# tenpy/cyten

Measured on AMD Instinct MI355X. Metric: block-sparse tdot+SVD GFLOP/s (fp64), higher is better.
Workload: dtype f64

## Files before the change

cyten_amd/csrc/jacobi_engine.hip:

```cpp
#include "jacobi_engine.h"
#include "jacobi_plan.h"

#include <algorithm>
#include <cmath>
#include <cstdlib>

namespace cyb {
namespace {

typedef double d4 __attribute__((ext_vector_type(4)));
typedef double d2 __attribute__((ext_vector_type(2)));
#define GLOBAL_AS __attribute__((address_space(1)))
typedef const GLOBAL_AS d2* gc2;
typedef const GLOBAL_AS d2* gcp2;
typedef GLOBAL_AS double* gp;

constexpr int GS = JP + 2;
constexpr int QS = JP + 16;
constexpr int GK = 64;
constexpr int XS = GK + 2;
constexpr int NT = 256;
constexpr int NPAIR = JP / 2;
static_assert(JP == 32, "the wave tiling below assumes 32 x 32 pair problems");

// ... 513 lines not shown
                double* Xr = which ? Ur : Hr;
                double* Xi = which ? Ui : Hi;
                const double c = rot[k * 4], sn = rot[k * 4 + 1], fr = rot[k * 4 + 2], fi = -rot[k * 4 + 3];
                const double pr_ = Xr[row * CS + p], pi_ = Xi[row * CS + p], qr_ = Xr[row * CS + q], qi_ = Xi[row * CS + q];
                const double tr = fr * qr_ - fi * qi_, ti = fr * qi_ + fi * qr_;
                Xr[row * CS + p] = c * pr_ - sn * tr;
                Xi[row * CS + p] = c * pi_ - sn * ti;
                Xr[row * CS + q] = sn * pr_ + c * tr;
                Xi[row * CS + q] = sn * pi_ + c * ti;
            }
            __builtin_amdgcn_fence(__ATOMIC_RELEASE, "wavefront");
            __builtin_amdgcn_wave_barrier();
        }
    for (int e = lane; e < CJ * CJ; e += 64) {
        const int a = e / CJ, b = e % CJ;
        const double x = Ur[a * CS + b], y = Ui[a * CS + b];
        Vout[(2 * a) * VS + 2 * b] = x;
        Vout[(2 * a) * VS + 2 * b + 1] = -y;
        Vout[(2 * a + 1) * VS + 2 * b] = y;
        Vout[(2 * a + 1) * VS + 2 * b + 1] = x;
    }
    if (lane < CJ) {
        const double lam = Hr[lane * CS + lane];
        Gdiag[(2 * lane) * GS + 2 * lane] = lam;
        Gdiag[(2 * lane + 1) * GS + 2 * lane + 1] = lam;
    }
}

struct SScratch {
    double* gpart;
    unsigned int* ticket;
    unsigned int* ready;
    unsigned int* err;
    const int2* wgmap;
    const int2* wgent;
    unsigned long long* stamps;
    int stamp_round;
    int n_sweeps, n_mats;
    unsigned int* arrive;
    int* nsw;
    unsigned int* readyJ;
    int defer_j;
    unsigned long long* gran;
    int gran_np;
    int cross_every, cross_min_nb;
};
constexpr int SW_MAX_ENT = 64;

constexpr int SW_UN = 8;
constexpr int SW_PRE = 6;
constexpr int SW_GRAN_U64 = 2 * JP * JP;
constexpr unsigned int SW_GRAN_BYTES = 8u * SW_GRAN_U64;
static_assert(SW_GRAN_BYTES == kPlanGranBytes, "granule regions of jacobi_plan.h");
constexpr int SWEEP_XREG = (4 * JP * GS > JP * GS + 2 * JP * VS) ? 4 * JP * GS : JP * GS + 2 * JP * VS;
constexpr int SWEEP_LDS_DOUBLES = JP * GS + SWEEP_XREG + 2 * JP * QS + 8;
constexpr size_t SWEEP_LDS_BYTES = 88 * 1024;
static_assert((size_t)SWEEP_LDS_DOUBLES * 8 + 1024 <= SWEEP_LDS_BYTES, "LDS request of the sweep kernel");
constexpr int SWEEP_WG_PER_CU = 1;

typedef unsigned int u32x2 __attribute__((ext_vector_type(2)));
union Q8 {
    u32x2 u;
    double d;
};

template <int SLEEP = 1>
__device__ __forceinline__ bool spin_until(const unsigned int* word, unsigned int target, unsigned int* err)
{
    const unsigned long long t0 = wall_clock64();
    unsigned int it = 0;
    while (__hip_atomic_load(word, __ATOMIC_RELAXED, __HIP_MEMORY_SCOPE_AGENT) < target) {
        __builtin_amdgcn_s_sleep(SLEEP);
        if ((++it & 63u) == 0u) {
            if (__hip_atomic_load(err, __ATOMIC_RELAXED, __HIP_MEMORY_SCOPE_AGENT) != 0u) return false;
            if (wall_clock64() - t0 > 100000000ull) {
                __hip_atomic_store(err, 1u, __ATOMIC_RELAXED, __HIP_MEMORY_SCOPE_AGENT);
                return false;
            }
        }
    }
    return true;
}

template <int SLEEP = 1>
__device__ __forceinline__ bool spin_until2(const unsigned int* word0, const unsigned int* word1, unsigned int target, unsigned int* err)
{
    const unsigned long long t0 = wall_clock64();
    unsigned int it = 0;
    for (;;) {
        const unsigned int v0 = __hip_atomic_load(word0, __ATOMIC_RELAXED, __HIP_MEMORY_SCOPE_AGENT);
        const unsigned int v1 = __hip_atomic_load(word1, __ATOMIC_RELAXED, __HIP_MEMORY_SCOPE_AGENT);
        if ((v0 >= target) & (v1 >= target)) return true;
        __builtin_amdgcn_s_sleep(SLEEP);
        if ((++it & 63u) == 0u) {
            if (__hip_atomic_load(err, __ATOMIC_RELAXED, __HIP_MEMORY_SCOPE_AGENT) != 0u) return false;
            if (wall_clock64() - t0 > 100000000ull) {
                __hip_atomic_store(err, 1u, __ATOMIC_RELAXED, __HIP_MEMORY_SCOPE_AGENT);
                return false;
            }
        }
    }
}
template <bool RORD>
__device__ __forceinline__ bool spin_pair(const unsigned int* word0, const unsigned int* word1, unsigned int target, unsigned int* err)
{
    if constexpr (RORD) return spin_until2(word0, word1, target, err);
    else return spin_until(word0, target, err) && spin_until(word1, target, err);
}

__device__ __forceinline__ void sweep_update_j(const __amdgpu_buffer_rsrc_t rsJ, const double* Qm, int P, int Q, int nvp, int j_begin,
                                               int nJ, int wave, int lane)
{
    const int un = lane & 15, ukq = lane >> 4;
    const double* ap0 = Qm + (lane >> 4) * QS + (lane & 15);
    const double* ap1 = ap0 + 16;
    double a0[JP / 4], a1[JP / 4];
#pragma unroll
    for (int kk = 0; kk < JP / 4; ++kk) {
        a0[kk] = ap0[kk * 4 * QS];
        a1[kk] = ap1[kk * 4 * QS];
    }
    auto off_of = [&](int c, int k) { return (unsigned int)(((int64_t)xrow(k, P, Q) * nvp + (j_begin + c) * 64 + wave * 16 + un) * 8); };
    auto load = [&](double (&x)[JP / 4], int c) {
#pragma unroll
        for (int kk = 0; kk < JP / 4; ++kk) {
            Q8 q;
            q.u = __builtin_amdgcn_raw_buffer_load_b64(rsJ, off_of(c, 4 * kk + ukq), 0, 16);
            x[kk] = q.d;
        }
    };
    double xb[JP / 4], xn[JP / 4];
    if (nJ > 0) load(xb, 0);
    for (int c = 0; c < nJ; ++c) {
        if (c + 1 < nJ) load(xn, c + 1);
        d4 acc[2] = {d4{0.0, 0.0, 0.0, 0.0}, d4{0.0, 0.0, 0.0, 0.0}};
#pragma unroll
        for (int kk = 0; kk < JP / 4; ++kk) {
            acc[0] = __builtin_amdgcn_mfma_f64_16x16x4f64(a0[kk], xb[kk], acc[0], 0, 0, 0);
            acc[1] = __builtin_amdgcn_mfma_f64_16x16x4f64(a1[kk], xb[kk], acc[1], 0, 0, 0);
        }
#pragma unroll
        for (int i = 0; i < 2; ++i)
#pragma unroll
            for (int q = 0; q < 4; ++q) {
                Q8 v;
                v.d = acc[i][q];
                __builtin_amdgcn_raw_buffer_store_b64(v.u, rsJ, off_of(c, i * 16 + (lane >> 4) + 4 * q), 0, 16);
            }
#pragma unroll
        for (int kk = 0; kk < JP / 4; ++kk) xb[kk] = xn[kk];
    }
}

template <bool CPLX, bool RORD, bool GRAN>
__global__ void __launch_bounds__(NT, 1)
jacobi_sweep_kernel(const RPair* __restrict__ pairs, int max_inner, unsigned long long* __restrict__ offmax_bits, SScratch sc)
{
    extern __shared__ __attribute__((aligned(16))) double rsm[];
    double* Gs = rsm;
    double* G2 = Gs + JP * GS;
    double* Va = G2 + JP * GS;
    double* Vb = Va + JP * VS;
    double* Xc = G2;
    double* Qs0 = G2 + SWEEP_XREG;
    double* Qs1 = Qs0 + JP * QS;
    double* red = Qs1 + JP * QS;
    int* ibase = reinterpret_cast<int*>(red + 8);
    int* perm = ibase;
    int* zrow = ibase + JP;
    int* zout = ibase + 2 * JP;
    int* flags = ibase + 3 * JP;
    int* edone = flags + 4;

    const int tid = threadIdx.x;
    const int lane = tid & 63, wave = tid >> 6;
    const int2 went = sc.wgent ? sc.wgent[blockIdx.x] : make_int2((int)blockIdx.x, (int)blockIdx.x + 1);
    int max_rounds = 0;
    for (int e = went.x; e < went.y; ++e) max_rounds = max(max_rounds, pairs[sc.wgmap[e].x].nb - 1);
    const int n_sw = sc.n_sweeps;
    const bool one_entry = went.y - went.x == 1;
    int pendP = -1, pendQ = -1, pend_ground = 0;
    if (n_sw > 1) {
        if (tid < SW_MAX_ENT) edone[tid] = 0;
        __syncthreads();
    }
    for (int sw = 0; sw < n_sw; ++sw) {
    for (int round = 0; round < max_rounds; ++round)
    for (int ent = went.x; ent < went.y; ++ent) {
    const int2 wm = sc.wgmap[ent];
    const int pi = wm.x, part = wm.y;
    const RPair mt = pairs[pi];
    if (round >= mt.nb - 1) continue;
    if (n_sw > 1 && edone[ent - went.x]) continue;
    const int ground = sw * (mt.nb - 1) + round;
    const int G = mt.pad[0];
    unsigned int* ready = sc.ready + mt.pad[1];
    unsigned int* readyJ = sc.readyJ + mt.pad[1];
    unsigned int* ticket = sc.ticket + pi;
    double* Qs = (ground & 1) ? Qs1 : Qs0;
    const unsigned int pbytes = JP * JP * 8;
    const __amdgpu_buffer_rsrc_t rsW = __builtin_amdgcn_make_buffer_rsrc(mt.W, 0, (int)((size_t)mt.nvp * mt.lenp * 8), 0x00020000);
    const __amdgpu_buffer_rsrc_t rsJ =
        __builtin_amdgcn_make_buffer_rsrc(mt.J ? mt.J : mt.W, 0, mt.J ? (int)((size_t)mt.nvp * mt.nvp * 8) : 0, 0x00020000);
    const int cw = mt.lenp / 64, cj = mt.J ? mt.nvp / 64 : 0;
    const int w_begin = (int)((int64_t)part * cw / G), w_end = (int)((int64_t)(part + 1) * cw / G);
    const int j_begin = (int)((int64_t)part * cj / G), j_end = (int)((int64_t)(part + 1) * cj / G);
    const int nW = w_end - w_begin, nJ = j_end - j_begin;
    const bool defer = sc.defer_j && one_entry && G > 1 && nJ > 0 && round < mt.nb - 2;
    const int ct = defer ? nW : nW + nJ;
    const int pre_limit = (sc.defer_j && G > 1) ? min(ct, nW) : ct;
    const int un = lane & 15, ukq = lane >> 4;
#define SWEEP_STAMP(k)                                                                                            \
    do {                                                                                                          \
        if (sc.stamps && tid == 0 && round == sc.stamp_round) sc.stamps[(size_t)blockIdx.x * 8 + (k)] = wall_clock64(); \
    } while (0)

    {
        int P, Q;
        circle_pair(mt.nb, round, mt.slot, P, Q);
        if (P > Q) {
            const int t = P;
            P = Q;
            Q = t;
        }
        SWEEP_STAMP(0);
        __syncthreads();
        if (ground > 0) {
            if (tid == 0) {
                flags[1] = spin_pair<RORD>(ready + (size_t)P * G + part, ready + (size_t)Q * G + part, (unsigned int)ground, sc.err) ? 1 : 0;
            }
            __syncthreads();
            if (!flags[1]) return;
        }
        SWEEP_STAMP(1);
        if constexpr (GRAN) {
            if (tid == 0) flags[3] = 0;
        }
        auto chunk_off = [&](int c, int k, bool& in_w) -> unsigned int {
            in_w = c < nW;
            const int ld = in_w ? mt.lenp : mt.nvp;
            const int cc = in_w ? w_begin + c : j_begin + (c - nW);
            return (unsigned int)(((int64_t)xrow(k, P, Q) * ld + cc * 64 + wave * 16 + un) * 8);
        };
        auto chunk_load = [&](int c, int k) -> double {
            bool in_w;
            const unsigned int off = chunk_off(c, k, in_w);
            Q8 q;
            q.u = in_w ? __builtin_amdgcn_raw_buffer_load_b64(rsW, off, 0, 16) : __builtin_amdgcn_raw_buffer_load_b64(rsJ, off, 0, 16);
            return q.d;
        };
        double xpre[SW_PRE][JP / 4];
        auto issue_xpre = [&]() {
#pragma unroll
            for (int c = 0; c < SW_PRE; ++c) {
                if (c < pre_limit) {
#pragma unroll
                    for (int kk = 0; kk < JP / 4; ++kk) xpre[c][kk] = chunk_load(c, 4 * kk + ukq);
                }
            }
        };
        {
            const int ld = mt.lenp;
            d4 acc00 = d4{0.0, 0.0, 0.0, 0.0}, acc01 = acc00, acc11 = acc00;
            const int r = lane & 15, g2 = 2 * (lane >> 4);
            const unsigned int o0 = (unsigned int)(((int64_t)xrow(r, P, Q) * ld + g2) * 8);
            const unsigned int o1 = (unsigned int)(((int64_t)xrow(r + 16, P, Q) * ld + g2) * 8);
            const int c_begin = 8 * w_begin, c_end = 8 * w_end;
            constexpr int UN = SW_UN;
            d2 x0[UN], x1[UN], n0[UN], n1[UN];
            auto load = [&](d2 (&a0)[UN], d2 (&a1)[UN], int c0) {
#pragma unroll
                for (int u = 0; u < UN; ++u) {
                    const int c = min(c0 + 4 * u, c_end - 1);
                    Q16 qa, qb;
                    qa.u = __builtin_amdgcn_raw_buffer_load_b128(rsW, o0 + (unsigned int)c * 64u, 0, 16);
                    qb.u = __builtin_amdgcn_raw_buffer_load_b128(rsW, o1 + (unsigned int)c * 64u, 0, 16);
                    a0[u] = qa.d;
                    a1[u] = qb.d;
                }
            };
            auto gram = [&](const d2 (&a0)[UN], const d2 (&a1)[UN], int c0) {
#pragma unroll
                for (int u = 0; u < UN; ++u) {
                    if (c0 + 4 * u < c_end) {
                        acc00 = __builtin_amdgcn_mfma_f64_16x16x4f64(a0[u].x, a0[u].x, acc00, 0, 0, 0);
                        acc01 = __builtin_amdgcn_mfma_f64_16x16x4f64(a0[u].x, a1[u].x, acc01, 0, 0, 0);
                        acc11 = __builtin_amdgcn_mfma_f64_16x16x4f64(a1[u].x, a1[u].x, acc11, 0, 0, 0);
                        acc00 = __builtin_amdgcn_mfma_f64_16x16x4f64(a0[u].y, a0[u].y, acc00, 0, 0, 0);
                        acc01 = __builtin_amdgcn_mfma_f64_16x16x4f64(a0[u].y, a1[u].y, acc01, 0, 0, 0);
                        acc11 = __builtin_amdgcn_mfma_f64_16x16x4f64(a1[u].y, a1[u].y, acc11, 0, 0, 0);
                    }
                }
            };
            if constexpr (RORD) {
                int c0 = c_begin + wave;
                if (c0 < c_end) {
                    load(x0, x1, c0);
                    for (;;) {
                        if (c0 + 4 * UN < c_end) {
                            load(n0, n1, c0 + 4 * UN);
                            gram(x0, x1, c0);
                        } else {
                            gram(x0, x1, c0);
                            break;
                        }
                        c0 += 4 * UN;
                        if (c0 + 4 * UN < c_end) {
                            load(x0, x1, c0 + 4 * UN);
                            gram(n0, n1, c0);
                        } else {
                            gram(n0, n1, c0);
                            break;
                        }
                        c0 += 4 * UN;
                    }
                }
            } else {
            if (c_begin + wave < c_end) load(x0, x1, c_begin + wave);
            issue_xpre();
            for (int c0 = c_begin + wave; c0 < c_end; c0 += 4 * UN) {
                const bool more = c0 + 4 * UN < c_end;
                if (more) load(n0, n1, c0 + 4 * UN);
                gram(x0, x1, c0);
                if (more) {
#pragma unroll
                    for (int u = 0; u < UN; ++u) {
                        x0[u] = n0[u];
                        x1[u] = n1[u];
                    }
                }
            }
            }
            double* wpart = Xc + wave * (JP * GS);
#pragma unroll
            for (int q = 0; q < 4; ++q) {
                const int rr = (lane >> 4) + 4 * q, cc = lane & 15;
                wpart[rr * GS + cc] = acc00[q];
                wpart[rr * GS + 16 + cc] = acc01[q];
                wpart[(16 + cc) * GS + rr] = acc01[q];
                wpart[(16 + rr) * GS + 16 + cc] = acc11[q];
            }
        }
        __syncthreads();
        SWEEP_STAMP(2);
        if constexpr (RORD) __builtin_amdgcn_s_waitcnt(0x0F70);
        {
            const int gi = tid >> 3, gj = 4 * (tid & 7);
            d2 lo = d2{0.0, 0.0}, hi = d2{0.0, 0.0};
#pragma unroll
            for (int w = 0; w < 4; ++w) {
                const double* src = Xc + w * (JP * GS) + gi * GS + gj;
                lo.x += src[0];
                lo.y += src[1];
                hi.x += src[2];
                hi.y += src[3];
            }
            const __amdgpu_buffer_rsrc_t rs_all = __builtin_amdgcn_make_buffer_rsrc(
                sc.gpart + ((size_t)pi * 2 + (size_t)(ground & 1)) * RGMAX * (JP * JP), 0, (int)(pbytes * G), 0x00020000);
            const unsigned int gtag = (unsigned int)(ground + 1);
            GLOBAL_AS unsigned long long* gran_pair =
                (GLOBAL_AS unsigned long long*)sc.gran +
                ((size_t)(mt.pad[1] - sc.gran_np) + (size_t)(2 * mt.slot + (ground & 1)) * (size_t)G) * SW_GRAN_U64;
            if constexpr (GRAN) {
                if (G > 1) {
                    GLOBAL_AS unsigned long long* mine = gran_pair + (size_t)part * SW_GRAN_U64 + (size_t)(wave * 512 + lane);
                    const double v[4] = {lo.x, lo.y, hi.x, hi.y};
#pragma unroll
                    for (int k = 0; k < 4; ++k) {
                        __hip_atomic_store(mine + 128 * k, ((unsigned long long)gtag << 32) | (unsigned int)__double2loint(v[k]), __ATOMIC_RELAXED,
                                           __HIP_MEMORY_SCOPE_AGENT);
                        __hip_atomic_store(mine + 128 * k + 64, ((unsigned long long)gtag << 32) | (unsigned int)__double2hiint(v[k]), __ATOMIC_RELAXED,
                                           __HIP_MEMORY_SCOPE_AGENT);
                    }
                }
            } else if (G > 1) {
                Q16 a, b;
                a.d = lo;
                b.d = hi;
                const unsigned int off = (unsigned int)part * pbytes + (unsigned int)tid * 32u;
                __builtin_amdgcn_raw_buffer_store_b128(a.u, rs_all, off, 0, 16);
                __builtin_amdgcn_raw_buffer_store_b128(b.u, rs_all, off + 16u, 0, 16);
                asm volatile("s_waitcnt vmcnt(0)" ::: "memory");
                __syncthreads();
                if (tid == 0) __hip_atomic_fetch_add(ticket, 1u, __ATOMIC_RELAXED, __HIP_MEMORY_SCOPE_AGENT);
            }
            if constexpr (RORD) issue_xpre();
            if (G > 1) {
                if (pendP >= 0) {
                    if (tid == 0) {
                        flags[1] = spin_pair<RORD>(readyJ + (size_t)pendP * G + part, readyJ + (size_t)pendQ * G + part, (unsigned int)pend_ground, sc.err) ? 1 : 0;
                    }
                    __syncthreads();
                    if (!flags[1]) return;
                    sweep_update_j(rsJ, (pend_ground & 1) ? Qs1 : Qs0, pendP, pendQ, mt.nvp, j_begin, nJ, wave, lane);
                    asm volatile("s_waitcnt vmcnt(0)" ::: "memory");
                    __syncthreads();
                    if (tid == 0) {
                        __hip_atomic_store(readyJ + (size_t)pendP * G + part, (unsigned int)(pend_ground + 1), __ATOMIC_RELAXED, __HIP_MEMORY_SCOPE_AGENT);
                        __hip_atomic_store(readyJ + (size_t)pendQ * G + part, (unsigned int)(pend_ground + 1), __ATOMIC_RELAXED, __HIP_MEMORY_SCOPE_AGENT);
                    }
                    pendP = -1;
                }
                const d2 own_lo = lo, own_hi = hi;
                lo = d2{0.0, 0.0};
                hi = d2{0.0, 0.0};
                if constexpr (GRAN) {
                    const __amdgpu_buffer_rsrc_t rs_gran = __builtin_amdgcn_make_buffer_rsrc((unsigned long long*)gran_pair, 0, (int)(SW_GRAN_BYTES * G), 0x00020000);
                    const unsigned long long t0 = wall_clock64();
                    unsigned int it = 0, passes = 0;
                    bool good = true;
                    for (int g0 = 0; g0 < G && good; g0 += 4) {
                        u32x2 w[4][8];
                        for (;;) {
                            asm volatile("" ::: "memory");
                            unsigned int bad = 0u;
#pragma unroll
                            for (int g = 0; g < 4; ++g) {
                                if (g0 + g < G && g0 + g != part) {
#pragma unroll
                                    for (int j = 0; j < 8; ++j)
                                        w[g][j] = __builtin_amdgcn_raw_buffer_load_b64(rs_gran, (unsigned int)(wave * 4096 + lane * 8) + 512u * j, (g0 + g) * (int)SW_GRAN_BYTES, 16);
                                }
                            }
#pragma unroll
                            for (int g = 0; g < 4; ++g) {
                                if (g0 + g < G && g0 + g != part) {
#pragma unroll
                                    for (int j = 0; j < 8; ++j) bad |= w[g][j][1] ^ gtag;
                                }
                            }
                            ++passes;
                            if (__all(bad == 0u)) break;
                            __builtin_amdgcn_s_sleep(1);
                            if ((++it & 63u) == 0u) {
                                if (__hip_atomic_load(sc.err, __ATOMIC_RELAXED, __HIP_MEMORY_SCOPE_AGENT) != 0u) good = false;
                                else if (wall_clock64() - t0 > 100000000ull) {
                                    __hip_atomic_store(sc.err, 1u, __ATOMIC_RELAXED, __HIP_MEMORY_SCOPE_AGENT);
                                    good = false;
                                }
                                if (!good) break;
                            }
                        }
                        if (!good) break;
#pragma unroll
                        for (int g = 0; g < 4; ++g) {
                            if (g0 + g == part) {
                                lo += own_lo;
                                hi += own_hi;
                            } else if (g0 + g < G) {
                                lo.x += __hiloint2double((int)w[g][1][0], (int)w[g][0][0]);
                                lo.y += __hiloint2double((int)w[g][3][0], (int)w[g][2][0]);
                                hi.x += __hiloint2double((int)w[g][5][0], (int)w[g][4][0]);
                                hi.y += __hiloint2double((int)w[g][7][0], (int)w[g][6][0]);
                            }
                        }
                    }
                    if (!good && lane == 0) flags[3] = 1;
                    if (sc.stamps && tid == 0 && round == sc.stamp_round) sc.stamps[(size_t)blockIdx.x * 8 + 7] = passes;
                } else {
                if (tid == 0) flags[1] = spin_until(ticket, (unsigned int)G * (unsigned int)(ground + 1), sc.err) ? 1 : 0;
                __syncthreads();
                if (!flags[1]) return;
                for (int g0 = 0; g0 < G; g0 += 4) {
                    Q16 pa[4], pb[4];
#pragma unroll
                    for (int g = 0; g < 4; ++g) {
                        if (g0 + g < G) {
                            pa[g].u = __builtin_amdgcn_raw_buffer_load_b128(rs_all, (unsigned int)(g0 + g) * pbytes + (unsigned int)tid * 32u, 0, 16);
                            pb[g].u = __builtin_amdgcn_raw_buffer_load_b128(rs_all, (unsigned int)(g0 + g) * pbytes + (unsigned int)tid * 32u + 16u, 0, 16);
                        }
                    }
#pragma unroll
                    for (int g = 0; g < 4; ++g) {
                        if (g0 + g < G) {
                            lo += pa[g].d;
                            hi += pb[g].d;
                        }
                    }
                }
                }
            }
            double* dst = Gs + gi * GS + gj;
            dst[0] = lo.x;
            dst[1] = lo.y;
            dst[2] = hi.x;
            dst[3] = hi.y;
        }
        __syncthreads();
        if constexpr (GRAN) {
            if (G > 1 && flags[3]) return;
        }
        SWEEP_STAMP(3);
        if (tid == 0) flags[0] = 0;
        __syncthreads();
        if (tid < JP) {
            double g = Gs[tid * GS + tid];
            if constexpr (CPLX) g = fmax(g, Gs[(tid ^ 1) * GS + (tid ^ 1)]);
            const int z = (g > 0.0 && g <= mt.thr2) ? 1 : 0;
            zrow[tid] = z;
            perm[tid] = tid;
            if (z) flags[0] = 1;
        }
        __syncthreads();
        const bool any_null = flags[0] != 0;
        if (any_null) {
            for (int e = tid; e < JP * JP; e += NT) {
                const int i = e / JP, j = e % JP;
                if (zrow[i] || zrow[j]) Gs[i * GS + j] = 0.0;
            }
            __syncthreads();
        }
        const double off = gram_offmax(Gs, red, tid);
        if (part == 0 && tid == 0) atomicMax(offmax_bits + (size_t)sw * sc.n_mats + mt.mat, (unsigned long long)__double_as_longlong(off));
        const bool skip = off <= mt.tol && !any_null;
        if (!skip) {
            double* Ga = Gs;
            double* Gb = G2;
            double* Vc = Va;
            double* Vn = Vb;
            bool pos_is_interleaved = false;
            const int cross_k = sc.cross_every > 0 ? sc.cross_every : max(4, (mt.nb + 2) / 4);
            const bool cross = sc.cross_every != 0 && !any_null && mt.nb >= sc.cross_min_nb && (round % cross_k) != 0;
            if constexpr (CPLX) {
                if (tid < 64) hermitian_pivot_solve(Gs, G2, Vb, Va, Gs, max_inner, tid, 0.25 * mt.tol * mt.tol, cross);
                __syncthreads();
            } else {
            auto cpos = [](int i) { return i < JB ? 2 * i : 2 * (i - JB) + 1; };
            pos_is_interleaved = cross;
            if (cross) {
                for (int e = tid; e < JP * JP; e += NT) {
                    const int i = e / JP, j = e % JP;
                    Gb[cpos(i) * GS + cpos(j)] = Ga[i * GS + j];
                }
                for (int e = tid; e < JP * VS; e += NT) Va[e] = (cpos(e / VS) == (e % VS)) ? 1.0 : 0.0;
                double* t = Ga;
                Ga = Gb;
                Gb = t;
            } else
                for (int e = tid; e < JP * VS; e += NT) Va[e] = ((e / VS) == (e % VS)) ? 1.0 : 0.0;
            __syncthreads();
            {
                const int pr = tid >> 4, pc = tid & 15;
                const int r0 = 2 * pr, c0 = 2 * pc;
                const int dr0 = cross ? r0 : ring_next(r0), dr1 = cross ? ((r0 + 3) & (JP - 1)) : ring_next(r0 + 1);
                const int dc0 = cross ? c0 : ring_next(c0), dc1 = cross ? ((c0 + 3) & (JP - 1)) : ring_next(c0 + 1);
                const int n_steps = cross ? JB : JP - 1;
                for (int sweep = 0; sweep < (off <= mt.tol ? 0 : max_inner); ++sweep) {
                    for (int r = 0; r < n_steps; ++r) {
                        const d2 g0 = *reinterpret_cast<const d2*>(Ga + r0 * GS + c0);
                        const d2 g1 = *reinterpret_cast<const d2*>(Ga + (r0 + 1) * GS + c0);
                        const d2 ac = *reinterpret_cast<const d2*>(Ga + c0 * GS + c0);
                        const double dc = Ga[(c0 + 1) * GS + c0 + 1];
                        const d2 v0 = *reinterpret_cast<const d2*>(Vc + r0 * VS + c0);
                        const d2 v1 = *reinterpret_cast<const d2*>(Vc + (r0 + 1) * VS + c0);
                        double c1, s1, c2, s2;
                        jacobi_rot_bf(ac.x, dc, ac.y, c2, s2, 0.25 * mt.tol * mt.tol);
                        const int rsrc = (lane & 48) | pr;
                        c1 = __shfl(c2, rsrc);
                        s1 = __shfl(s2, rsrc);
                        const double hik = c1 * g0.x - s1 * g1.x, hil = c1 * g0.y - s1 * g1.y;
                        const double hjk = s1 * g0.x + c1 * g1.x, hjl = s1 * g0.y + c1 * g1.y;
                        double nik = c2 * hik - s2 * hil, nil = s2 * hik + c2 * hil;
                        double njk = c2 * hjk - s2 * hjl, njl = s2 * hjk + c2 * hjl;
                        if (pr == pc) {
                            nil = 0.0;
                            njk = 0.0;
                        }
                        Gb[dr0 * GS + dc0] = nik;
                        Gb[dr0 * GS + dc1] = nil;
                        Gb[dr1 * GS + dc0] = njk;
                        Gb[dr1 * GS + dc1] = njl;
                        Vn[r0 * VS + dc0] = c2 * v0.x - s2 * v0.y;
                        Vn[r0 * VS + dc1] = s2 * v0.x + c2 * v0.y;
                        Vn[(r0 + 1) * VS + dc0] = c2 * v1.x - s2 * v1.y;
                        Vn[(r0 + 1) * VS + dc1] = s2 * v1.x + c2 * v1.y;
                        __syncthreads();
                        double* t = Ga;
                        Ga = Gb;
                        Gb = t;
                        t = Vc;
                        Vc = Vn;
                        Vn = t;
                    }
                    if (sweep + 1 < max_inner) {
                        const double off_in = gram_offmax(Ga, red, tid);
                        if (off_in <= 0.25 * mt.tol) break;
                    }
                }
            }
            }
            __syncthreads();
            SWEEP_STAMP(4);
            if (off > mt.tol && tid < 64) {
                const int li = lane & (JP - 1);
                const int li_idx = pos_is_interleaved ? ((li & 1) ? JB + (li >> 1) : (li >> 1)) : li;
                const double g = xrow(li_idx, P, Q) < mt.nv ? Ga[li * GS + li] : -1.0e300;
                const int glo = __double2loint(g), ghi = __double2hiint(g);
                int rk = 0;
#pragma unroll
                for (int j = 0; j < JP; ++j) {
                    const double gj = __hiloint2double(__builtin_amdgcn_readlane(ghi, j), __builtin_amdgcn_readlane(glo, j));
                    rk += (gj > g || (gj == g && j < li)) ? 1 : 0;
                }
                if (lane < JP) perm[rk] = lane;
            }
            __syncthreads();
            for (int e = tid; e < JP * JP; e += NT) {
                const int k = e / JP, m = e % JP;
                Qs[k * QS + m] = Vc[k * VS + perm[m]];
            }
            if (tid < JP) {
                const int pp = perm[tid];
                zout[tid] = zrow[pos_is_interleaved ? ((pp & 1) ? JB + (pp >> 1) : (pp >> 1)) : pp];
            }
            __syncthreads();
            SWEEP_STAMP(5);
            if (ct > nW) {
                if (tid == 0) {
                    flags[1] = spin_pair<RORD>(readyJ + (size_t)P * G + part, readyJ + (size_t)Q * G + part, (unsigned int)ground, sc.err) ? 1 : 0;
                }
                __syncthreads();
                if (!flags[1]) return;
#pragma unroll
                for (int c = 0; c < SW_PRE; ++c) {
                    if (c >= pre_limit && c < ct) {
#pragma unroll
                        for (int kk = 0; kk < JP / 4; ++kk) xpre[c][kk] = chunk_load(c, 4 * kk + ukq);
                    }
                }
            }
            if (ct > 0) {
                const double* ap0 = Qs + (lane >> 4) * QS + (lane & 15);
                const double* ap1 = ap0 + 16;
                double a0[JP / 4], a1[JP / 4];
#pragma unroll
                for (int kk = 0; kk < JP / 4; ++kk) {
                    a0[kk] = ap0[kk * 4 * QS];
                    a1[kk] = ap1[kk * 4 * QS];
                }
                int zr[2][4];
#pragma unroll
                for (int i = 0; i < 2; ++i)
#pragma unroll
                    for (int q = 0; q < 4; ++q) zr[i][q] = zout[i * 16 + (lane >> 4) + 4 * q];
                auto apply = [&](int c, const double (&xb)[JP / 4]) {
                    d4 acc[2] = {d4{0.0, 0.0, 0.0, 0.0}, d4{0.0, 0.0, 0.0, 0.0}};
#pragma unroll
                    for (int kk = 0; kk < JP / 4; ++kk) {
                        acc[0] = __builtin_amdgcn_mfma_f64_16x16x4f64(a0[kk], xb[kk], acc[0], 0, 0, 0);
                        acc[1] = __builtin_amdgcn_mfma_f64_16x16x4f64(a1[kk], xb[kk], acc[1], 0, 0, 0);
                    }
                    const bool zero_null = c < nW;
#pragma unroll
                    for (int i = 0; i < 2; ++i)
#pragma unroll
                        for (int q = 0; q < 4; ++q) {
                            const int row = i * 16 + (lane >> 4) + 4 * q;
                            bool in_w;
                            const unsigned int o = chunk_off(c, row, in_w);
                            Q8 v;
                            v.d = (zero_null && zr[i][q]) ? 0.0 : acc[i][q];
                            if (in_w) __builtin_amdgcn_raw_buffer_store_b64(v.u, rsW, o, 0, 16);
                            else __builtin_amdgcn_raw_buffer_store_b64(v.u, rsJ, o, 0, 16);
                        }
                };
#pragma unroll
                for (int c = 0; c < SW_PRE; ++c)
                    if (c < ct) apply(c, xpre[c]);
                if (ct > SW_PRE) {
                    double xb[JP / 4], xn[JP / 4];
#pragma unroll
                    for (int kk = 0; kk < JP / 4; ++kk) xb[kk] = chunk_load(SW_PRE, 4 * kk + ukq);
                    if constexpr (RORD) {
                        auto fetch = [&](double (&x)[JP / 4], int c) {
#pragma unroll
                            for (int kk = 0; kk < JP / 4; ++kk) x[kk] = chunk_load(c, 4 * kk + ukq);
                        };
                        for (int c = SW_PRE;;) {
                            if (c + 1 < ct) {
                                fetch(xn, c + 1);
                                apply(c, xb);
                            } else {
                                apply(c, xb);
                                break;
                            }
                            ++c;
                            if (c + 1 < ct) {
                                fetch(xb, c + 1);
                                apply(c, xn);
                            } else {
                                apply(c, xn);
                                break;
                            }
                            ++c;
                        }
                    } else
                    for (int c = SW_PRE; c < ct; ++c) {
                        if (c + 1 < ct) {
#pragma unroll
                            for (int kk = 0; kk < JP / 4; ++kk) xn[kk] = chunk_load(c + 1, 4 * kk + ukq);
                        }
                        apply(c, xb);
#pragma unroll
                        for (int kk = 0; kk < JP / 4; ++kk) xb[kk] = xn[kk];
                    }
                }
            }
        }
        if (defer && !skip) {
            pendP = P;
            pendQ = Q;
            pend_ground = ground;
        }
        asm volatile("s_waitcnt vmcnt(0)" ::: "memory");
        __syncthreads();
        if (tid == 0) {
            if (skip && nJ > 0) {
                if constexpr (RORD) (void)spin_until2(readyJ + (size_t)P * G + part, readyJ + (size_t)Q * G + part, (unsigned int)ground, sc.err);
                else {
                    (void)spin_until(readyJ + (size_t)P * G + part, (unsigned int)ground, sc.err);
                    (void)spin_until(readyJ + (size_t)Q * G + part, (unsigned int)ground, sc.err);
                }
            }
            __hip_atomic_store(ready + (size_t)P * G + part, (unsigned int)(ground + 1), __ATOMIC_RELAXED, __HIP_MEMORY_SCOPE_AGENT);
            __hip_atomic_store(ready + (size_t)Q * G + part, (unsigned int)(ground + 1), __ATOMIC_RELAXED, __HIP_MEMORY_SCOPE_AGENT);
            if (!(defer && !skip)) {
                __hip_atomic_store(readyJ + (size_t)P * G + part, (unsigned int)(ground + 1), __ATOMIC_RELAXED, __HIP_MEMORY_SCOPE_AGENT);
                __hip_atomic_store(readyJ + (size_t)Q * G + part, (unsigned int)(ground + 1), __ATOMIC_RELAXED, __HIP_MEMORY_SCOPE_AGENT);
            }
            if (n_sw > 1 && round == mt.nb - 2) __hip_atomic_fetch_add(sc.arrive + mt.mat, 1u, __ATOMIC_RELAXED, __HIP_MEMORY_SCOPE_AGENT);
        }
        SWEEP_STAMP(6);
    }
    }
    if (n_sw == 1) break;
    __syncthreads();
    if (tid == 0) {
        int all = 1, ok = 1;
        for (int ent = went.x; ent < went.y && ok; ++ent) {
            if (edone[ent - went.x]) continue;
            const int2 wm = sc.wgmap[ent];
            const RPair mt = pairs[wm.x];
            const unsigned int entries = (unsigned int)(mt.nb / 2) * (unsigned int)mt.pad[0];
            if (!spin_until<32>(sc.arrive + mt.mat, entries * (unsigned int)(sw + 1), sc.err)) {
                ok = 0;
                break;
            }
            const double off = __longlong_as_double((long long)__hip_atomic_load(offmax_bits + (size_t)sw * sc.n_mats + mt.mat, __ATOMIC_RELAXED, __HIP_MEMORY_SCOPE_AGENT));
            const double prev = sw ? __longlong_as_double((long long)__hip_atomic_load(offmax_bits + (size_t)(sw - 1) * sc.n_mats + mt.mat,
                                                                                      __ATOMIC_RELAXED, __HIP_MEMORY_SCOPE_AGENT))
                                   : 1e300;
            if (jacobi_sweep_done(off, prev, mt.tol, sw + 1)) {
                edone[ent - went.x] = 1;
                if (mt.slot == 0 && wm.y == 0) sc.nsw[mt.mat] = sw + 1;
            } else all = 0;
        }
        flags[1] = ok;
        flags[2] = all;
    }
    __syncthreads();
    if (!flags[1] || flags[2]) return;
    }
#undef SWEEP_STAMP
}


struct JSwitches {
    bool no_sweep;
    bool per_sweep;
    bool one_launch_all;
    bool trace;
    bool stamps;
    bool no_predict;
    bool gran_exchange;
    bool round_order;
    bool no_defer_j;
    bool cross_small;
    int g;
    int inner;
    int cross;
    int cross_min_nb;
};
const JSwitches& switches()
{
    static const JSwitches s = [] {
        auto on = [](const char* name) { return getenv(name) != nullptr; };
        auto num = [](const char* name, int dflt) { return getenv(name) ? atoi(getenv(name)) : dflt; };
        JSwitches w;
        w.no_sweep = on("CYB_JACOBI_NOSWEEP");
        w.per_sweep = on("CYB_JACOBI_PERSWEEP");
        w.one_launch_all = on("CYB_JACOBI_ONELAUNCH");
        w.trace = on("CYB_JACOBI_TRACE");
        w.stamps = on("CYB_JACOBI_STAMPS");
        w.no_predict = on("CYB_JACOBI_NOPREDICT");
        w.gran_exchange = num("CYB_JACOBI_EXCHANGE", 1) != 0;
        w.round_order = num("CYB_JACOBI_ROUND_ORDER", 1) != 0;
        w.no_defer_j = on("CYB_JACOBI_NODEFERJ");
        w.cross_small = on("CYB_JACOBI_CROSS_SMALL");
        w.g = num("CYB_JACOBI_G", 0);
        w.inner = num("CYB_JACOBI_INNER", 0);
        w.cross = num("CYB_JACOBI_CROSS", -1);
        w.cross_min_nb = num("CYB_JACOBI_CROSS_MINNB", 0);
        return w;
    }();
    return s;
}

struct SweepCall {
    int n;
    int n_sw_dev;
    size_t w_off;
    size_t b_off;
    bool cplx;
};

struct SweepList {
    std::vector<int> order;
    std::vector<JWork> wl;
    std::vector<PlanMat> pm;
    int max_nb = 0;
    bool any_j = false;
    bool big_ok = true;
};
SweepList build_work_list(const std::vector<JMat>& h_mats, const std::vector<int>& active)
{
    SweepList l;
    l.order = active;
    std::stable_sort(l.order.begin(), l.order.end(), [&](int a, int b) { return h_mats[(size_t)a].nb > h_mats[(size_t)b].nb; });
    for (int m : l.order) {
        const JMat& jm = h_mats[(size_t)m];
        l.max_nb = std::max(l.max_nb, jm.nb);
        for (int k = 0; k < jm.nb / 2; ++k) l.wl.push_back(JWork{m, k});
        l.pm.push_back(PlanMat{jm.nb, jm.nvp, jm.lenp, jm.J != nullptr || jm.rec_j != 0});
        l.any_j = l.any_j || jm.J != nullptr;
        l.big_ok = l.big_ok && (size_t)jm.nvp * (size_t)std::max(jm.lenp, jm.nvp) * 8 < ((size_t)1 << 31);
    }
    return l;
}

struct SweepScratch {
    void* base = nullptr;
    size_t zero_bytes;
    unsigned long long* d_off;
    unsigned int* d_err;
    unsigned int* d_ready;
    unsigned long long* d_gran;
    double* gpart;
    JScratch split;
    size_t split_cnt_bytes;
};
int carve_scratch(cyb_ctx_t ctx, const SweepLayout& L, size_t b_off, SweepScratch& s)
{
    const size_t np = L.np;
    const size_t b_gpart = sizeof(double) * np * RGMAX * JP * JP, b_q = sizeof(double) * np * JP * JP;
    const size_t b_z = sizeof(int32_t) * np * JP, b_f = (sizeof(int32_t) * np + 15) / 16 * 16, b_c = (sizeof(unsigned int) * np + 15) / 16 * 16;
    void* wsp = nullptr;
    const int status = ctx->workspace(L.zero_bytes + L.gran_reserved + 2 * b_gpart + 2 * (b_q + b_z + b_f) + b_c + 1024, &wsp, 2);
    if (status != CYB_OK) return status;
    char* bp = static_cast<char*>(wsp);
    s.base = wsp;
    s.zero_bytes = L.zero_bytes;
    s.d_off = reinterpret_cast<unsigned long long*>(bp);
    s.d_err = reinterpret_cast<unsigned int*>(bp + b_off);
    s.d_ready = reinterpret_cast<unsigned int*>(bp + b_off + 16);
    s.d_gran = reinterpret_cast<unsigned long long*>(bp + L.zero_bytes);
    bp += L.zero_bytes + L.gran_reserved;
    s.gpart = reinterpret_cast<double*>(bp);
    bp += 2 * b_gpart;
    s.split.gpart = s.gpart;
    for (int h = 0; h < 2; ++h) {
        s.split.qout[h] = reinterpret_cast<double*>(bp);
        bp += b_q;
    }
    for (int h = 0; h < 2; ++h) {
        s.split.zout[h] = reinterpret_cast<int32_t*>(bp);
        bp += b_z;
    }
    for (int h = 0; h < 2; ++h) {
        s.split.flag[h] = reinterpret_cast<int32_t*>(bp);
        bp += b_f;
    }
    s.split.cnt = reinterpret_cast<unsigned int*>(bp);
    s.split_cnt_bytes = b_c;
    return CYB_OK;
}

struct ImageCache {
    std::vector<int> order, G;
    uint64_t at = 0;
    void* img = nullptr;
};
int descriptor_image(cyb_ctx_t ctx, ImageCache& cache, const std::vector<JMat>& h_mats, const SweepList& list, const SweepPlan& plan)
{
    uint64_t& cached_at = cache.at;
    if (cache.img && list.order == cache.order && plan.G == cache.G && ctx->n_uploads - cached_at < (uint64_t)cyb_ctx_s::kSlots / 2 - 1)
        return CYB_OK;
    const SweepLayout& L = plan.layout;
    std::vector<char> img(L.image_bytes);
    RPair* rp = reinterpret_cast<RPair*>(img.data());
    int2* wgmap = reinterpret_cast<int2*>(img.data() + L.map_off);
    size_t k = 0, e = 0;
    for (size_t i = 0; i < list.order.size(); ++i) {
        const JMat& jm = h_mats[(size_t)list.order[i]];
        for (int slot = 0; slot < jm.nb / 2; ++slot, ++k) {
            RPair& q = rp[k];
            q.W = jm.W;
            q.J = jm.J;
            q.tol = jm.tol;
            q.thr2 = jm.thr2;
            q.nvp = jm.nvp;
            q.lenp = jm.lenp;
            q.nb = jm.nb;
            q.nv = jm.nv;
            q.mat = list.order[i];
            q.slot = slot;
            q.pad[0] = plan.G[i];
            q.pad[1] = L.flag_base[i];
            for (int g = 0; g < plan.G[i]; ++g) wgmap[e++] = make_int2((int)k, g);
        }
    }
    if (!plan.share.ranges.empty()) memcpy(img.data() + L.ent_off, plan.share.ranges.data(), sizeof(PlanRange) * plan.share.ranges.size());
    const int status = ctx->upload(img.data(), img.size(), &cache.img);
    if (status != CYB_OK) return status;
    cache.order = list.order;
    cache.G = plan.G;
    cached_at = ctx->n_uploads;
    return CYB_OK;
}

typedef void (*sweep_fn_t)(const RPair*, int, unsigned long long*, SScratch);
int sweep_kernel_for(bool cplx, sweep_fn_t& fn)
{
    static const sweep_fn_t sweep_fns[2][2][2] = {
        {{jacobi_sweep_kernel<false, false, false>, jacobi_sweep_kernel<false, false, true>},
         {jacobi_sweep_kernel<false, true, false>, jacobi_sweep_kernel<false, true, true>}},
        {{jacobi_sweep_kernel<true, false, false>, jacobi_sweep_kernel<true, false, true>},
         {jacobi_sweep_kernel<true, true, false>, jacobi_sweep_kernel<true, true, true>}}};
    const JSwitches& sw = switches();
    static const sweep_fn_t sweep_fn[2] = {sweep_fns[0][sw.round_order ? 1 : 0][sw.gran_exchange ? 1 : 0],
                                           sweep_fns[1][sw.round_order ? 1 : 0][sw.gran_exchange ? 1 : 0]};
    static bool attr_set = false;
    if (!attr_set) {
        for (int c = 0; c < 2; ++c)
            if (hipFuncSetAttribute(reinterpret_cast<const void*>(sweep_fn[c]), hipFuncAttributeMaxDynamicSharedMemorySize,
                                    (int)SWEEP_LDS_BYTES) != hipSuccess) {
                set_error("jacobi: cannot reserve %zu bytes of LDS for the sweep kernel", SWEEP_LDS_BYTES);
                return CYB_ERR_HIP;
            }
        attr_set = true;
    }
    fn = sweep_fn[cplx ? 1 : 0];
    return CYB_OK;
}

void print_sweep_stamps(hipStream_t st, const unsigned long long* d_stamps, const SweepList& list, const SweepPlan& plan, int sweep, int stamp_round)
{
    const size_t entries = plan.layout.entries;
    std::vector<unsigned long long> hs(8 * entries);
    if (hipMemcpyAsync(hs.data(), d_stamps, sizeof(unsigned long long) * hs.size(), hipMemcpyDeviceToHost, st) != hipSuccess ||
        hipStreamSynchronize(st) != hipSuccess)
        return;
    double acc[6] = {0, 0, 0, 0, 0, 0}, passes = 0;
    const int cntw = list.pm[0].nb / 2 * plan.G[0];
    const bool swept = switches().gran_exchange && plan.G[0] > 1;
    for (size_t b = 0; b < (size_t)cntw; ++b) {
        for (int k = 0; k < 6; ++k) acc[k] += (double)(hs[8 * b + k + 1] - hs[8 * b + k]) * 0.01;
        if (swept) passes += (double)hs[8 * b + 7];
    }
    if (cntw)
        fprintf(stderr, "[jacobi sweep stamps] sweep %d round %d, largest matrix (G=%d, %d workgroups of %zu): wait %.2f load+gram %.2f "
                        "exch %.2f defl+eig %.2f sort %.2f upd+publish %.2f us, granule passes %.1f\n",
                sweep, stamp_round, plan.G[0], cntw, entries, acc[0] / cntw, acc[1] / cntw, acc[2] / cntw, acc[3] / cntw, acc[4] / cntw,
                acc[5] / cntw, passes / cntw);
}

int launch_sweep(cyb_ctx_t ctx, const std::vector<JMat>& h_mats, const SweepList& list, const SweepPlan& plan, const SweepScratch& s,
                 ImageCache& cache, const SweepCall& call, int sweep, int max_inner, bool& one_launch)
{
    const JSwitches& sw = switches();
    const SweepLayout& L = plan.layout;
    hipStream_t st = ctx->stream;
    int status = descriptor_image(ctx, cache, h_mats, list, plan);
    if (status != CYB_OK) return status;
    sweep_fn_t fn = nullptr;
    status = sweep_kernel_for(call.cplx, fn);
    if (status != CYB_OK) return status;
    const std::vector<PlanRange>& ranges = plan.share.ranges;
    static unsigned long long* d_stamps = nullptr;
    if (sw.stamps && !d_stamps && hipMalloc(reinterpret_cast<void**>(&d_stamps), sizeof(unsigned long long) * 8 * 2048) != hipSuccess) d_stamps = nullptr;
    SScratch ss;
    ss.gpart = s.gpart;
    ss.ticket = s.d_ready;
    ss.ready = s.d_ready;
    ss.readyJ = s.d_ready + L.ready_reserved;
    ss.defer_j = sw.no_defer_j ? 0 : 1;
    ss.cross_every = (max_inner == 1 || sw.cross_small) ? sw.cross : 0;
    ss.cross_min_nb = sw.cross_min_nb;
    ss.err = s.d_err;
    ss.wgmap = reinterpret_cast<const int2*>(static_cast<char*>(cache.img) + L.map_off);
    ss.wgent = ranges.empty() ? nullptr : reinterpret_cast<const int2*>(static_cast<char*>(cache.img) + L.ent_off);
    ss.stamps = ranges.empty() ? d_stamps : nullptr;
    ss.stamp_round = std::min(3, list.max_nb - 2);
    size_t max_ent = 1;
    for (const PlanRange& we : ranges) max_ent = std::max(max_ent, (size_t)(we.end - we.begin));
    one_launch = call.n_sw_dev > 1 && sweep == 1 && max_ent <= (size_t)SW_MAX_ENT;
    ss.n_sweeps = one_launch ? call.n_sw_dev : 1;
    ss.n_mats = call.n;
    ss.arrive = reinterpret_cast<unsigned int*>(s.d_off + call.w_off);
    ss.nsw = reinterpret_cast<int*>(ss.arrive + call.n);
    ss.gran = s.d_gran;
    ss.gran_np = (int)L.np;
    if (L.gran_used > L.gran_reserved) {
        set_error("jacobi: %zu bytes of granule regions exceed the %zu reserved", L.gran_used, L.gran_reserved);
        return CYB_ERR_INVALID;
    }
    if (hipMemsetAsync(s.base, 0, s.zero_bytes + L.gran_used, st) != hipSuccess) return CYB_ERR_HIP;
    const size_t n_wg = ranges.empty() ? L.entries : ranges.size();
    hipLaunchKernelGGL(fn, dim3((unsigned)n_wg), dim3(NT), SWEEP_LDS_BYTES, st, static_cast<const RPair*>(cache.img), max_inner, s.d_off, ss);
    if (ss.stamps && L.entries <= 2048) print_sweep_stamps(st, d_stamps, list, plan, sweep, ss.stamp_round);
    return CYB_OK;
}

int launch_rounds_split(cyb_ctx_t ctx, const std::vector<JMat>& h_mats, const SweepList& list, const SweepScratch& s, int max_inner)
{
    hipStream_t st = ctx->stream;
    const JScratch& sc = s.split;
    const int g_env = switches().g;
    if (hipMemsetAsync(s.base, 0, s.zero_bytes, st) != hipSuccess) return CYB_ERR_HIP;
    void *d_mats_v = nullptr, *d_wl = nullptr;
    int status = ctx->upload(h_mats.data(), sizeof(JMat) * h_mats.size(), &d_mats_v);
    if (status == CYB_OK) status = ctx->upload(list.wl.data(), sizeof(JWork) * list.wl.size(), &d_wl);
    if (status != CYB_OK) return status;
    const JMat* d_mats = static_cast<const JMat*>(d_mats_v);
    if (hipMemsetAsync(sc.cnt, 0, s.split_cnt_bytes, st) != hipSuccess) return CYB_ERR_HIP;
    int pend_round = -1;
    size_t pend_cnt = 0;
    for (int r = 0; r < list.max_nb - 1; ++r) {
        size_t cnt = 0;
        for (int m : list.order) {
            if (h_mats[(size_t)m].nb - 1 > r) cnt += (size_t)h_mats[(size_t)m].nb / 2;
            else break;
        }
        if (cnt == 0) break;
        const int slots = 2 * ctx->n_cu;
        int G = g_env > 0 ? g_env : ((size_t)2 * cnt <= (size_t)slots ? 2 : 1);
        G = std::min(G, RGMAX);
        const int U = (int)std::min<size_t>(16, std::max<size_t>(1, (size_t)(3 * ctx->n_cu) / cnt));
        const int buf = r & 1;
        const int n_gram = (int)(cnt * G);
        int UJ = 1;
        size_t n_jwg = 0;
        if (pend_round >= 0) {
            const long long free_slots = (long long)slots - (long long)n_gram;
            UJ = (int)std::max<long long>(1, std::min<long long>(8, free_slots / (long long)pend_cnt));
            n_jwg = pend_cnt * (size_t)UJ;
        }
        hipLaunchKernelGGL(jacobi_gram_kernel, dim3((unsigned)(n_gram + n_jwg)), dim3(NT), 0, st, d_mats,
                           static_cast<const JWork*>(d_wl), r, G, max_inner, s.d_off, sc, buf, n_gram, pend_round, UJ);
        const bool defer = list.any_j;
        hipLaunchKernelGGL(jacobi_update_kernel, dim3((unsigned)(cnt * U)), dim3(NT), 0, st, d_mats,
                           static_cast<const JWork*>(d_wl), r, U, sc, buf, 1, defer ? 0 : 1);
        pend_round = defer ? r : -1;
        pend_cnt = cnt;
    }
    if (pend_round >= 0) {
        const int U = (int)std::min<size_t>(16, std::max<size_t>(1, (size_t)(3 * ctx->n_cu) / pend_cnt));
        hipLaunchKernelGGL(jacobi_update_kernel, dim3((unsigned)(pend_cnt * U)), dim3(NT), 0, st, d_mats,
                           static_cast<const JWork*>(d_wl), pend_round, U, sc, pend_round & 1, 0, 1);
    }
    return CYB_OK;
}

int read_back(cyb_ctx_t ctx, const SweepScratch& s, std::vector<unsigned long long>& h_off, size_t b_off)
{
    if (ctx->d2h(h_off.data(), s.d_off, b_off + 16) != CYB_OK) {
        set_error("jacobi: reading the convergence flags failed: %s", hipGetErrorString(hipGetLastError()));
        return CYB_ERR_HIP;
    }
    unsigned int h_err = 0;
    memcpy(&h_err, reinterpret_cast<const char*>(h_off.data()) + b_off, sizeof(unsigned int));
    if (h_err) {
        set_error("jacobi round kernel: a workgroup waited more than a second for the Gram partials of its pair "
                  "(partner workgroup not resident?)");
        return CYB_ERR_HIP;
    }
    return CYB_OK;
}

void sweep_verdicts(const std::vector<JMat>& h_mats, const std::vector<unsigned long long>& h_off, int sweep, std::vector<int>& active,
                    std::vector<double>& prev_off, std::vector<int32_t>& sweeps_out)
{
    const JSwitches& sw = switches();
    std::vector<int> still;
// ... 95 lines not shown
```

Before: 5899.

## Fold Jacobi sweep setup passes into fewer barriers via round-pass kernel variant

Adds an RP template variant of the sweep kernel, on by default. It writes the Gram tile straight into interleaved order, computes the off-diagonal max from register-held Gram values, and initialises V in the same pass as null detection. The rank sort now runs across all waves, and the GEMM reads V through the permutation instead of materialising Qs first; Qs is built only when the J update is deferred. The aim is to cut several __syncthreads barriers and LDS copy passes per pair round, at the cost of gathered LDS reads and more code paths.

```diff
diff --git a/cyten_amd/csrc/jacobi_engine.hip b/cyten_amd/csrc/jacobi_engine.hip
--- a/cyten_amd/csrc/jacobi_engine.hip
+++ b/cyten_amd/csrc/jacobi_engine.hip
@@ -689,10 +689,11 @@
     }
 }
 
-template <bool CPLX, bool RORD, bool GRAN>
+template <bool CPLX, bool RORD, bool GRAN, bool RP>
 __global__ void __launch_bounds__(NT, 1)
 jacobi_sweep_kernel(const RPair* __restrict__ pairs, int max_inner, unsigned long long* __restrict__ offmax_bits, SScratch sc)
 {
+    static_assert(!RP || (RORD && GRAN), "the folded passes exist for the default round order and exchange only");
     extern __shared__ __attribute__((aligned(16))) double rsm[];
     double* Gs = rsm;
     double* G2 = Gs + JP * GS;
@@ -773,6 +774,15 @@
         if constexpr (GRAN) {
             if (tid == 0) flags[3] = 0;
         }
+        if constexpr (RP) {
+            if (tid == 0) flags[0] = 0;
+        }
+        const int cross_k = sc.cross_every > 0 ? sc.cross_every : max(4, (mt.nb + 2) / 4);
+        const bool cross_terms = sc.cross_every != 0 && mt.nb >= sc.cross_min_nb && (round % cross_k) != 0;
+        auto cpos = [](int i) { return i < JB ? 2 * i : 2 * (i - JB) + 1; };
+        auto cidx = [](int p) { return (p & 1) ? JB + (p >> 1) : (p >> 1); };
+        const bool ilv = RP && !CPLX && cross_terms;
+        double gv[4] = {0.0, 0.0, 0.0, 0.0};
         auto chunk_off = [&](int c, int k, bool& in_w) -> unsigned int {
             in_w = c < nW;
             const int ld = in_w ? mt.lenp : mt.nvp;
@@ -1017,17 +1027,72 @@
                 }
                 }
             }
+            if constexpr (RP) {
+                gv[0] = lo.x;
+                gv[1] = lo.y;
+                gv[2] = hi.x;
+                gv[3] = hi.y;
+                double* dst = Gs + (ilv ? cpos(gi) * GS + cpos(gj) : gi * GS + gj);
+                const int ds = ilv ? 2 : 1;
+#pragma unroll
+                for (int k = 0; k < 4; ++k) dst[k * ds] = gv[k];
+            } else {
             double* dst = Gs + gi * GS + gj;
             dst[0] = lo.x;
             dst[1] = lo.y;
             dst[2] = hi.x;
             dst[3] = hi.y;
+            }
         }
         __syncthreads();
         if constexpr (GRAN) {
             if (G > 1 && flags[3]) return;
         }
         SWEEP_STAMP(3);
+        double off;
+        bool any_null;
+        if constexpr (RP) {
+            const int gi = tid >> 3, gj = 4 * (tid & 7);
+            double m = 0.0;
+            if (gi < gj + 3) {
+                const double gii = Gs[(ilv ? cpos(gi) : gi) * (GS + 1)];
+#pragma unroll
+                for (int k = 0; k < 4; ++k) {
+                    const int j = gj + k;
+                    if (gi < j) {
+                        const double den = gii * Gs[(ilv ? cpos(j) : j) * (GS + 1)];
+                        if (den > 0.0) m = fmax(m, fabs(gv[k]) * rsqrt(den));
+                    }
+                }
+            }
+            m = wave_max(m);
+            if (lane == 0) red[wave] = m;
+            if (tid < JP) {
+                double g = Gs[(ilv ? cpos(tid) : tid) * (GS + 1)];
+                if constexpr (CPLX) g = fmax(g, Gs[(tid ^ 1) * (GS + 1)]);
+                const int z = (g > 0.0 && g <= mt.thr2) ? 1 : 0;
+                zrow[tid] = z;
+                perm[tid] = tid;
+                if (z) flags[0] = 1;
+            }
+            if constexpr (!CPLX) {
+                for (int e = tid; e < JP * VS; e += NT) {
+                    const int k = e / VS;
+                    Va[e] = ((ilv ? cpos(k) : k) == (e % VS)) ? 1.0 : 0.0;
+                }
+            }
+            __syncthreads();
+            off = fmax(fmax(red[0], red[1]), fmax(red[2], red[3]));
+            any_null = flags[0] != 0;
+            if (any_null) {
+#pragma unroll
+                for (int k = 0; k < 4; ++k) Gs[gi * GS + gj + k] = (zrow[gi] || zrow[gj + k]) ? 0.0 : gv[k];
+                if (ilv)
+                    for (int e = tid; e < JP * VS; e += NT) Va[e] = ((e / VS) == (e % VS)) ? 1.0 : 0.0;
+                __syncthreads();
+                off = gram_offmax(Gs, red, tid);
+            }
+        } else {
         if (tid == 0) flags[0] = 0;
         __syncthreads();
         if (tid < JP) {
@@ -1039,7 +1104,7 @@
             if (z) flags[0] = 1;
         }
         __syncthreads();
-        const bool any_null = flags[0] != 0;
+        any_null = flags[0] != 0;
         if (any_null) {
             for (int e = tid; e < JP * JP; e += NT) {
                 const int i = e / JP, j = e % JP;
@@ -1047,7 +1112,8 @@
             }
             __syncthreads();
         }
-        const double off = gram_offmax(Gs, red, tid);
+        off = gram_offmax(Gs, red, tid);
+        }
         if (part == 0 && tid == 0) atomicMax(offmax_bits + (size_t)sw * sc.n_mats + mt.mat, (unsigned long long)__double_as_longlong(off));
         const bool skip = off <= mt.tol && !any_null;
         if (!skip) {
@@ -1056,14 +1122,14 @@
             double* Vc = Va;
             double* Vn = Vb;
             bool pos_is_interleaved = false;
-            const int cross_k = sc.cross_every > 0 ? sc.cross_every : max(4, (mt.nb + 2) / 4);
-            const bool cross = sc.cross_every != 0 && !any_null && mt.nb >= sc.cross_min_nb && (round % cross_k) != 0;
+            const bool cross = cross_terms && !any_null;
             if constexpr (CPLX) {
                 if (tid < 64) hermitian_pivot_solve(Gs, G2, Vb, Va, Gs, max_inner, tid, 0.25 * mt.tol * mt.tol, cross);
                 __syncthreads();
             } else {
-            auto cpos = [](int i) { return i < JB ? 2 * i : 2 * (i - JB) + 1; };
             pos_is_interleaved = cross;
+            if constexpr (RP) {
+            } else {
             if (cross) {
                 for (int e = tid; e < JP * JP; e += NT) {
                     const int i = e / JP, j = e % JP;
@@ -1076,6 +1142,7 @@
             } else
                 for (int e = tid; e < JP * VS; e += NT) Va[e] = ((e / VS) == (e % VS)) ? 1.0 : 0.0;
             __syncthreads();
+            }
             {
                 const int pr = tid >> 4, pc = tid & 15;
                 const int r0 = 2 * pr, c0 = 2 * pc;
@@ -1126,11 +1193,37 @@
                 }
             }
             }
+            auto row_at = [&](int p) { return pos_is_interleaved ? cidx(p) : p; };
+            if constexpr (RP) {
+                SWEEP_STAMP(4);
+                if (off > mt.tol) {
+                    const int li = 8 * wave + (lane >> 3), ch = lane & 7;
+                    auto key = [&](int p) { return xrow(row_at(p), P, Q) < mt.nv ? Ga[p * GS + p] : -1.0e300; };
+                    const double g = key(li);
+                    int rk = 0;
+#pragma unroll
+                    for (int k = 0; k < 4; ++k) {
+                        const int j = 4 * ch + k;
+                        const double gj = key(j);
+                        rk += (gj > g || (gj == g && j < li)) ? 1 : 0;
+                    }
+                    rk += __shfl_xor(rk, 1);
+                    rk += __shfl_xor(rk, 2);
+                    rk += __shfl_xor(rk, 4);
+                    if (ch == 0) {
+                        perm[rk] = li;
+                        zout[rk] = zrow[row_at(li)];
+                    }
+                } else if (tid < JP)
+                    zout[tid] = zrow[row_at(tid)];
+                __syncthreads();
+                SWEEP_STAMP(5);
+            } else {
             __syncthreads();
             SWEEP_STAMP(4);
             if (off > mt.tol && tid < 64) {
                 const int li = lane & (JP - 1);
-                const int li_idx = pos_is_interleaved ? ((li & 1) ? JB + (li >> 1) : (li >> 1)) : li;
+                const int li_idx = row_at(li);
                 const double g = xrow(li_idx, P, Q) < mt.nv ? Ga[li * GS + li] : -1.0e300;
                 const int glo = __double2loint(g), ghi = __double2hiint(g);
                 int rk = 0;
@@ -1146,12 +1239,10 @@
                 const int k = e / JP, m = e % JP;
                 Qs[k * QS + m] = Vc[k * VS + perm[m]];
             }
-            if (tid < JP) {
-                const int pp = perm[tid];
-                zout[tid] = zrow[pos_is_interleaved ? ((pp & 1) ? JB + (pp >> 1) : (pp >> 1)) : pp];
-            }
+            if (tid < JP) zout[tid] = zrow[row_at(perm[tid])];
             __syncthreads();
             SWEEP_STAMP(5);
+            }
             if (ct > nW) {
                 if (tid == 0) {
                     flags[1] = spin_pair<RORD>(readyJ + (size_t)P * G + part, readyJ + (size_t)Q * G + part, (unsigned int)ground, sc.err) ? 1 : 0;
@@ -1167,13 +1258,14 @@
                 }
             }
             if (ct > 0) {
-                const double* ap0 = Qs + (lane >> 4) * QS + (lane & 15);
-                const double* ap1 = ap0 + 16;
+                const double* ap0 = RP ? Vc + (lane >> 4) * VS + perm[lane & 15] : Qs + (lane >> 4) * QS + (lane & 15);
+                const double* ap1 = RP ? Vc + (lane >> 4) * VS + perm[16 + (lane & 15)] : ap0 + 16;
+                constexpr int AS = RP ? VS : QS;
                 double a0[JP / 4], a1[JP / 4];
 #pragma unroll
                 for (int kk = 0; kk < JP / 4; ++kk) {
-                    a0[kk] = ap0[kk * 4 * QS];
-                    a1[kk] = ap1[kk * 4 * QS];
+                    a0[kk] = ap0[kk * 4 * AS];
+                    a1[kk] = ap1[kk * 4 * AS];
                 }
                 int zr[2][4];
 #pragma unroll
@@ -1243,6 +1335,14 @@
                     }
                 }
             }
+            if constexpr (RP) {
+                if (defer) {
+                    for (int e = tid; e < JP * JP; e += NT) {
+                        const int k = e / JP, m = e % JP;
+                        Qs[k * QS + m] = Vc[k * VS + perm[m]];
+                    }
+                }
+            }
         }
         if (defer && !skip) {
             pendP = P;
@@ -1311,6 +1411,7 @@
     bool no_predict;
     bool gran_exchange;
     bool round_order;
+    bool round_passes;
     bool no_defer_j;
     bool cross_small;
     int g;
@@ -1332,6 +1433,7 @@
         w.no_predict = on("CYB_JACOBI_NOPREDICT");
         w.gran_exchange = num("CYB_JACOBI_EXCHANGE", 1) != 0;
         w.round_order = num("CYB_JACOBI_ROUND_ORDER", 1) != 0;
+        w.round_passes = num("CYB_JACOBI_ROUND_PASSES", 1) != 0 && w.round_order && w.gran_exchange;
         w.no_defer_j = on("CYB_JACOBI_NODEFERJ");
         w.cross_small = on("CYB_JACOBI_CROSS_SMALL");
         w.g = num("CYB_JACOBI_G", 0);
@@ -1469,13 +1571,14 @@
 int sweep_kernel_for(bool cplx, sweep_fn_t& fn)
 {
     static const sweep_fn_t sweep_fns[2][2][2] = {
-        {{jacobi_sweep_kernel<false, false, false>, jacobi_sweep_kernel<false, false, true>},
-         {jacobi_sweep_kernel<false, true, false>, jacobi_sweep_kernel<false, true, true>}},
-        {{jacobi_sweep_kernel<true, false, false>, jacobi_sweep_kernel<true, false, true>},
-         {jacobi_sweep_kernel<true, true, false>, jacobi_sweep_kernel<true, true, true>}}};
+        {{jacobi_sweep_kernel<false, false, false, false>, jacobi_sweep_kernel<false, false, true, false>},
+         {jacobi_sweep_kernel<false, true, false, false>, jacobi_sweep_kernel<false, true, true, false>}},
+        {{jacobi_sweep_kernel<true, false, false, false>, jacobi_sweep_kernel<true, false, true, false>},
+         {jacobi_sweep_kernel<true, true, false, false>, jacobi_sweep_kernel<true, true, true, false>}}};
+    static const sweep_fn_t sweep_fns_rp[2] = {jacobi_sweep_kernel<false, true, true, true>, jacobi_sweep_kernel<true, true, true, true>};
     const JSwitches& sw = switches();
-    static const sweep_fn_t sweep_fn[2] = {sweep_fns[0][sw.round_order ? 1 : 0][sw.gran_exchange ? 1 : 0],
-                                           sweep_fns[1][sw.round_order ? 1 : 0][sw.gran_exchange ? 1 : 0]};
+    static const sweep_fn_t sweep_fn[2] = {sw.round_passes ? sweep_fns_rp[0] : sweep_fns[0][sw.round_order ? 1 : 0][sw.gran_exchange ? 1 : 0],
+                                           sw.round_passes ? sweep_fns_rp[1] : sweep_fns[1][sw.round_order ? 1 : 0][sw.gran_exchange ? 1 : 0]};
     static bool attr_set = false;
     if (!attr_set) {
         for (int c = 0; c < 2; ++c)
```

New measurement: 6122, median of 6. +3.8%, better.
